# LuletterSoul/RP-Style-Transfer

Hardware: AMD Instinct MI355X
Metric: stylized images/sec at 512×512, 1/2/4/8 MI355X; % HBM roofline (higher is better)
Workload: dtype fp32

## Files before the change

rp-style-transfer_amd/csrc/rpst_wino4q.hip:

```cpp
#include "rpst_conv.h"

#include <type_traits>

#ifndef RPST_W4Q_DBG
#define RPST_W4Q_DBG 0
#endif

namespace rpst {
namespace {

template <int PAD>
__device__ __forceinline__ void q_mfma(floatx4& acc, float a, float b) {
  if constexpr (PAD)
    asm volatile("s_nop 1\n\tv_mfma_f32_16x16x4_f32 %0, %1, %2, %0" : "+v"(acc) : "v"(a), "v"(b));
  else
    asm volatile("v_mfma_f32_16x16x4_f32 %0, %1, %2, %0" : "+v"(acc) : "v"(a), "v"(b));
}
__device__ __forceinline__ unsigned q_lds_addr(const float* p) {
  return (unsigned)(uintptr_t)(const __attribute__((address_space(3))) float*)p;
}
template <int OFF>
__device__ __forceinline__ void q_dma16(__amdgpu_buffer_rsrc_t r, unsigned m0, unsigned voff,
                                        int soff) {
  asm volatile("s_mov_b32 m0, %0\n\ts_nop 0\n\tbuffer_load_dwordx4 %1, %2, %3 offen offset:%4 lds"
               :: "s"(m0), "v"(voff), "s"(r), "s"(soff), "i"(OFF) : "memory");
}
__device__ __forceinline__ void q_dma4(__amdgpu_buffer_rsrc_t r, unsigned m0, unsigned voff,
                                       int soff) {
  asm volatile("s_mov_b32 m0, %0\n\ts_nop 0\n\tbuffer_load_dword %1, %2, %3 offen lds"
               :: "s"(m0), "v"(voff), "s"(r), "s"(soff) : "memory");
}
__device__ __forceinline__ void q_lds_barrier() {
  asm volatile("s_waitcnt lgkmcnt(0)" ::: "memory");
  __builtin_amdgcn_s_barrier();
}

template <int H>
__device__ __forceinline__ void q_bt3(float d0, float d1, float d2, float d3, float d4, float d5,
                                      float& u0, float& u1, float& u2) {
  if constexpr (H == 0) {
    const float A = fmaf(-4.f, d2, d4), B = fmaf(-4.f, d1, d3);
    u0 = fmaf(4.f, d0, fmaf(-5.f, d2, d4));
    u1 = A + B;
    u2 = A - B;
  } else {
    const float C = d4 - d2, E = d3 - d1;
    u0 = fmaf(2.f, E, C);
    u1 = fmaf(-2.f, E, C);
    u2 = fmaf(4.f, d1, fmaf(-5.f, d3, d5));
  }
}

}

constexpr int kQCo = 64;
constexpr int kQTH = 8, kQTW = 64;
constexpr int kQXO = 4;
constexpr int kQPS = 72;
constexpr int kQCS = 768;
constexpr int kQWS = 9216;
constexpr int kQPAT = 4 * kQCS;
constexpr int kQNTH = 512;
constexpr int kQMaxCo = 512;
constexpr int kQWPI = 5;
constexpr int kQWide = 2, kQSlow = 6;
constexpr int kQDMA4 = 3, kQDMA = 12;
constexpr int kQRP = kQPS / 4;
constexpr int kQXS = 4 * 3 * 3 * 64 * 2;
constexpr int kQWG0 = 0;
constexpr int kQPG = 5;
constexpr int kQAhead = 3;
static_assert(10 * kQRP <= kQDMA4 * 64 && kQDMA4 * 256 <= kQCS, "16-B pieces in a channel");
static_assert(10 * kQPS <= kQDMA * 64 && kQDMA * 64 <= kQCS, "4-B pieces in a channel");
static_assert(2 * kQWide >= kQDMA4 && 2 * kQSlow >= kQDMA && 8 * kQWPI >= 36, "coverage");
static_assert(2 * kQXS <= kQWS, "the exchange fits a weight stage");
static_assert((2 * kQWS + 4 * kQPAT) * 4 + 1024 + kQSlow * kQNTH * 4 + 9 * kQMaxCo * 4 <= 163840,
              "LDS");

template <typename TW>
__global__ void wino4q_pack_kernel(const TW* __restrict__ w, float* __restrict__ pk, int Cout,
                                   int Cin, int K4, int64_t per, int64_t total, int64_t sco,
                                   int64_t sci, int64_t stap) {
  int64_t t = (int64_t)blockIdx.x * blockDim.x + threadIdx.x;
  if (t >= total) return;
  const int64_t img = t / per;
  pk += img * per;
  w += img * (int64_t)Cout * Cin * 9;
  t -= img * per;
  const int cb = (int)(t & 3);
  int64_t r = t >> 2;
  const int l = (int)(r & 63);
  r >>= 6;
  const int p = (int)(r % 9);
  r /= 9;
  const int q = (int)(r & 3);
  r >>= 2;
  const int ks = (int)(r % K4);
  const int ct = (int)(r / K4);
  const int i = 3 * (q >> 1) + p / 3, jj = 3 * (q & 1) + p % 3;
  const int co = ct * kQCo + cb * 16 + (l & 15);
  const int ci = ks * 4 + (l >> 4);
  float v = 0.f;
  if (co < Cout && ci < Cin) {
    const double G[6][3] = {{0.25, 0, 0},
                            {-1.0 / 6, -1.0 / 6, -1.0 / 6},
                            {-1.0 / 6, 1.0 / 6, -1.0 / 6},
                            {1.0 / 24, 1.0 / 12, 1.0 / 6},
                            {1.0 / 24, -1.0 / 12, 1.0 / 6},
                            {0, 0, 1}};
    const TW* g = w + co * sco + ci * sci;
    double acc = 0.0;
#pragma unroll
    for (int u = 0; u < 3; ++u)
#pragma unroll
      for (int s = 0; s < 3; ++s) acc += G[i][u] * (double)g[(u * 3 + s) * stap] * G[jj][s];
    v = (float)acc;
  }
  pk[t] = v;
}

size_t wino4q_packed_floats(int Cout, int Cin) {
  return (size_t)((Cout + kQCo - 1) / kQCo) * ((Cin + 3) / 4) * kQWS;
}

int wino4q_pack(const float* w, float* pk, int Cout, int Cin, hipStream_t st) {
  const int64_t t = (int64_t)wino4q_packed_floats(Cout, Cin);
  wino4q_pack_kernel<float><<<(unsigned)((t + 255) / 256), 256, 0, st>>>(
      w, pk, Cout, Cin, (Cin + 3) / 4, t, t, (int64_t)Cin * 9, 9, 1);
  return launch_status("wino4q_pack_kernel");
}

int wino4q_pack_mix(const double* wm, float* pk, int N, int Cout, int Cin, hipStream_t st) {
  const int64_t per = (int64_t)wino4q_packed_floats(Cout, Cin), tot = (int64_t)N * per;
  wino4q_pack_kernel<double><<<(unsigned)((tot + 255) / 256), 256, 0, st>>>(
      wm, pk, Cout, Cin, (Cin + 3) / 4, per, tot, Cin, 1, (int64_t)Cout * Cin);
  return launch_status("wino4q_pack_kernel(mix)");
}

__global__ void wino4q_fold_w_kernel(const float4* __restrict__ pk, float4* __restrict__ out,
                                     const float* __restrict__ aux, int N, int Cin, int K4,
                                     int64_t per4) {
  const int64_t t = (int64_t)blockIdx.x * blockDim.x + threadIdx.x;
  if (t >= (int64_t)N * per4) return;
  const int n = (int)(t / per4);
  const int64_t u = t - (int64_t)n * per4;
  const int l = (int)(u & 63);
  const int ks = (int)((u / (kQWS / 4)) % K4);
  const int ci = ks * 4 + (l >> 4);
  const int64_t nc = (int64_t)N * Cin, i = (int64_t)n * Cin + (ci < Cin ? ci : 0);
  const float sc = ci < Cin ? aux[3 * nc + i] / aux[2 * nc + i] : 0.f;
  const float4 v = pk[u];
  out[t] = make_float4(v.x * sc, v.y * sc, v.z * sc, v.w * sc);
}

int wino4q_fold_w(const float* pk, float* out, const float* aux, int N, int Cout, int Cin,
                  hipStream_t st) {
  const int64_t per4 = (int64_t)wino4q_packed_floats(Cout, Cin) / 4, n4 = (int64_t)N * per4;
  wino4q_fold_w_kernel<<<(unsigned)((n4 + 255) / 256), 256, 0, st>>>(
      reinterpret_cast<const float4*>(pk), reinterpret_cast<float4*>(out), aux, N, Cin,
      (Cin + 3) / 4, per4);
  return launch_status("wino4q_fold_w_kernel");
}

bool wino4q_applies(int Cin, int Cout, int in_op, const ConvMode& m) {
  const int min_cin = m.quarter == 2 ? 16 : 128;
  return m.quarter && m.precise != 2 && (in_op == RPST_IN_NONE || in_op == RPST_IN_UPSAMPLE2) &&
         Cout >= 64 && Cout <= kQMaxCo &&
         Cin >= min_cin && Cin % 16 == 0;
}

ConvTiling wino4q_tiling(ConvArgs& a) {
  a.Cout_pad = (a.Cout + kQCo - 1) / kQCo * kQCo;
  a.nchunks = (a.Cin + 3) / 4;
  a.tiles_x = (a.W + kQTW - 1) / kQTW;
  a.tiles_y = (a.H + kQTH - 1) / kQTH;
  a.co_tiles = a.Cout_pad / kQCo;
  a.stat_P = a.tiles_x * a.tiles_y * 2;
  a.cosplit = 1;
  return {(int64_t)a.tiles_x * a.tiles_y * a.N, kQNTH, 4, kQTH / 4, kQTW, true};
}

struct QEpi {
  int W, H, Cout, gy0, gx0, rows, n, sidx;
  bool vec, full, bst, edge, store, pool;
  float inv, slope;
  unsigned voff[4];
  float* out;
  float* oimg;
  unsigned obytes;
  const float* btab;
  float2* statp;
  int statP;
};

__device__ __forceinline__ QEpi q_epi_ctx(int wr, int tn) {
  const KArgs L = late_args();
  QEpi e;
  e.W = L->W;
  e.H = L->H;
  e.Cout = L->Cout;
  e.slope = L->relu == RPST_ACT_RELU ? 0.f : (L->relu == RPST_ACT_LRELU ? 0.2f : 1.f);
  int btx, bty;
  w4_tile((int)blockIdx.x / L->cosplit, L->tiles_x, L->tiles_y, btx, bty, e.n);
  const int bx0 = btx * kQTW;
  e.gy0 = bty * kQTH + 4 * wr;
  e.gx0 = bx0 + 4 * tn;
  e.vec = (e.W & 3) == 0 && e.gx0 + 3 < e.W;
  e.rows = max(0, min(4, e.H - e.gy0));
  const int cols = max(0, min(kQTW, e.W - bx0));
  e.inv = e.rows * cols > 0 ? __builtin_amdgcn_rcpf((float)(e.rows * cols)) : 0.f;
  e.full = e.rows == 4 && bx0 + kQTW <= e.W;
  e.edge = e.gy0 == 0 || e.gy0 + 4 >= e.H || bx0 == 0 || bx0 + kQTW >= e.W;
  e.out = L->out;
  const int64_t plane = (int64_t)e.H * e.W;
  e.pool = L->pool_out != 0;
  e.bst = !e.pool && (e.W & 3) == 0 && (int64_t)e.Cout * plane * 4 < (1LL << 31);
  e.oimg = e.out + (int64_t)e.n * e.Cout * plane;
  const bool keep = L->skip_from <= 0 || e.n < L->skip_from;
  e.obytes = keep ? (unsigned)(e.Cout * plane * 4) : 0u;
  e.store = keep;
#pragma unroll
  for (int yy = 0; yy < 4; ++yy)
    e.voff[yy] = (yy < e.rows && e.gx0 < e.W) ? (unsigned)(((e.gy0 + yy) * e.W + e.gx0) * 4)
                                             : 0x80000000u;
  e.btab = L->btab;
  e.statp = L->stat_part;
  e.statP = L->stat_P;
  e.sidx = (bty * L->tiles_x + btx) * 2 + wr;
  return e;
}

template <bool STATS, bool BTAB, bool RELU>
__device__ __forceinline__ void q_finish(const QEpi& e, int co, float (&Y)[16], int tn) {
  const int gy0 = e.gy0, gx0 = e.gx0, rows = e.rows, n = e.n;
  const bool cok = co < e.Cout;
  if constexpr (BTAB) {
    if (e.edge) {
      const float* bt = e.btab + (cok ? co : 0) * 9;
      float b9[9];
#pragma unroll
      for (int i = 0; i < 9; ++i) b9[i] = cok ? bt[i] : 0.f;
      const float b4 = b9[4];
#pragma unroll
      for (int i = 0; i < 9; ++i) b9[i] -= b4;
#pragma unroll
      for (int yy = 0; yy < 4; ++yy) {
        const int gy = gy0 + yy;
        const int rc = gy == 0 ? 0 : (gy >= e.H - 1 ? 2 : 1);
        const float l = rc == 0 ? b9[0] : (rc == 2 ? b9[6] : b9[3]);
        const float m = rc == 0 ? b9[1] : (rc == 2 ? b9[7] : b9[4]);
        const float r = rc == 0 ? b9[2] : (rc == 2 ? b9[8] : b9[5]);
#pragma unroll
        for (int xx = 0; xx < 4; ++xx) {
          const int gx = gx0 + xx;
          Y[yy * 4 + xx] += gx == 0 ? l : (gx >= e.W - 1 ? r : m);
        }
      }
    }
  }
#pragma unroll
  for (int i = 0; i < 16; ++i)
    Y[i] = __builtin_amdgcn_fmed3f(Y[i], RELU ? 0.f : e.slope * Y[i], __builtin_inff());
  float sum = 0.f;
  if constexpr (STATS) {
    if (e.full) {
#pragma unroll
      for (int i = 0; i < 16; ++i) sum += Y[i];
    } else {
#pragma unroll
      for (int yy = 0; yy < 4; ++yy)
#pragma unroll
        for (int xx = 0; xx < 4; ++xx) sum += (yy < rows && gx0 + xx < e.W) ? Y[yy * 4 + xx] : 0.f;
    }
  }
  if ((RPST_W4Q_DBG & 64) && e.statP > -7) {
  } else if (e.bst) {
    const auto ro = rsrc_or_zero(e.oimg, e.obytes, true);
    const unsigned cofs = cok ? (unsigned)co * (unsigned)(e.H * e.W) * 4u : 0x7fffffffu;
#pragma unroll
    for (int yy = 0; yy < 4; ++yy) {
      const floatx4 v = {Y[yy * 4], Y[yy * 4 + 1], Y[yy * 4 + 2], Y[yy * 4 + 3]};
      __builtin_amdgcn_raw_buffer_store_b128(__builtin_bit_cast(u32x4, v), ro,
                                             (int)(e.voff[yy] + cofs), 0, 0);
    }
  } else if (e.pool) {
    if (cok && e.store) {
      const int Ho = (e.H + 1) >> 1, Wo = (e.W + 1) >> 1;
      float* o = e.out + (((int64_t)n * e.Cout + co) * Ho + (gy0 >> 1)) * Wo + (gx0 >> 1);
#pragma unroll
      for (int py = 0; py < 2; ++py) {
        if (2 * py >= rows) continue;
        const bool y1 = 2 * py + 1 < rows;
        float pv[2];
#pragma unroll
        for (int px = 0; px < 2; ++px) {
          const bool x1 = gx0 + 2 * px + 1 < e.W;
          const float* t = Y + (2 * py) * 4 + 2 * px;
          float v = t[0];
          if (x1) v = fmaxf(v, t[1]);
          if (y1) v = fmaxf(v, t[4]);
          if (x1 && y1) v = fmaxf(v, t[5]);
          pv[px] = v;
        }
        if (gx0 + 3 < e.W && (Wo & 1) == 0) {
          *reinterpret_cast<float2*>(o + py * Wo) = make_float2(pv[0], pv[1]);
        } else {
          if (gx0 < e.W) o[py * Wo] = pv[0];
          if (gx0 + 2 < e.W) o[py * Wo + 1] = pv[1];
        }
      }
    }
  } else if (cok && e.store) {
    float* o = e.out + (((int64_t)n * e.Cout + co) * e.H + gy0) * e.W + gx0;
#pragma unroll
    for (int yy = 0; yy < 4; ++yy) {
      if (yy < rows) {
        if (e.vec) {
          *reinterpret_cast<float4*>(o + yy * e.W) =
              make_float4(Y[yy * 4], Y[yy * 4 + 1], Y[yy * 4 + 2], Y[yy * 4 + 3]);
        } else {
#pragma unroll
          for (int xx = 0; xx < 4; ++xx)
            if (gx0 + xx < e.W) o[yy * e.W + xx] = Y[yy * 4 + xx];
        }
      }
    }
  }
  if constexpr (STATS) {
    sum = row16_sum(sum);
    const float mean = sum * e.inv;
    float m2 = 0.f;
    if (e.full) {
#pragma unroll
      for (int i = 0; i < 16; ++i) m2 = fmaf(Y[i] - mean, Y[i] - mean, m2);
    } else {
#pragma unroll
      for (int yy = 0; yy < 4; ++yy)
#pragma unroll
        for (int xx = 0; xx < 4; ++xx) {
          const float dv = Y[yy * 4 + xx] - mean;
          m2 += (yy < rows && gx0 + xx < e.W) ? dv * dv : 0.f;
        }
    }
    m2 = row16_sum(m2);
    if (tn == 0 && cok)
      e.statp[((int64_t)n * e.statP + e.sidx) * e.Cout + co] = make_float2(mean, m2);
  }
}

template <int INOP, bool STATS, bool BTAB, bool RELU>
__global__ __launch_bounds__(kQNTH, 1) void wino4q_mfma_kernel(ConvArgs a) {
  __shared__ __attribute__((aligned(16))) float ws0[kQWS];
  __shared__ __attribute__((aligned(16))) float ws1[kQWS];
  __shared__ __attribute__((aligned(16))) float ps0[kQPAT];
  __shared__ __attribute__((aligned(16))) float ps1[kQPAT];
  __shared__ __attribute__((aligned(16))) float ps2[kQPAT];
  __shared__ __attribute__((aligned(16))) float ps3[kQPAT];
  __shared__ __attribute__((aligned(16))) float dummy[256];
  __shared__ unsigned poffs[kQSlow][kQNTH];
  __shared__ float btl[BTAB ? 9 * kQMaxCo : kQMaxCo];

  const int wave = __builtin_amdgcn_readfirstlane((int)threadIdx.x >> 6);
  const int lane = threadIdx.x & 63;
  const int k = lane >> 4, tn = lane & 15, wr = wave >> 2;

  int bid = (int)blockIdx.x;
  const int cog = bid % a.cosplit;
  bid /= a.cosplit;
  const int nct = a.co_tiles / a.cosplit, ct0 = cog * nct;
  int tx, ty, n;
  w4_tile(bid, a.tiles_x, a.tiles_y, tx, ty, n);
  const int K4 = a.nchunks, G = nct * K4;
  const int y0 = ty * kQTH, x0 = tx * kQTW;

  {
    const int nb = BTAB ? 9 * a.Cout : a.Cout;
    const float* src = BTAB ? a.btab + (int64_t)n * nb : a.bias;
    for (int i = threadIdx.x; i < nb; i += kQNTH) btl[i] = src ? src[i] : 0.f;
  }
  constexpr bool up = INOP == RPST_IN_UPSAMPLE2;
  const unsigned in_plane = up ? (unsigned)(a.Hs * a.Ws) : (unsigned)(a.H * a.W);
  const unsigned oob = a.Cin * in_plane * 4u;
  const float* in_img = conv_in_img(a, n, (int64_t)a.Cin * in_plane);
  const unsigned wbytes = (unsigned)(nct * K4 * kQWS) * 4u;
  const float* w_img = a.wpk + (int64_t)n * a.wstride + (int64_t)ct0 * K4 * kQWS;

  const int hf = wave & 1;
  const bool zp = a.pad == RPST_PAD_ZERO;
  const int rs = up ? a.Ws : a.W;
  const bool w4a = (a.W & 3) == 0;
  const bool wide = !up && ((x0 >= 1 && x0 + kQTW < a.W) || (w4a && x0 + kQTW <= a.W));
  const bool fixL = wide && w4a && !zp && x0 == 0;
  const bool fixR = wide && w4a && !zp && x0 + kQTW == a.W;
  unsigned poff[kQSlow];
  const int tid = threadIdx.x;
  if (wide) {
#pragma unroll
    for (int i = 0; i < kQWide; ++i) {
      const int p = kQWide * hf + i;
      const int f = 64 * p + lane, row = min(f / kQRP, 9), j = f - (f / kQRP) * kQRP;
      int y = y0 - 1 + row;
      const int xs = x0 - kQXO + 4 * j;
      const bool okx = !w4a || (xs >= 0 && xs + 3 < a.W);
      const bool ok = p < kQDMA4 && f < 10 * kQRP && resolve_bf(y, a.H, zp) && okx;
      poff[i] = ok ? ((unsigned)(y * rs) + (unsigned)xs) * 4u : oob;
    }
#pragma unroll
    for (int i = kQWide; i < kQSlow; ++i) poff[i] = oob;
  } else {
#pragma unroll
    for (int i = 0; i < kQSlow; ++i) {
      const int p = kQSlow * hf + i;
      const int f = 64 * p + lane;
      const int row = min(f / kQPS, 9), col = f - (f / kQPS) * kQPS;
      int y = y0 - 1 + row, x = x0 - kQXO + col;
      const bool oky = resolve_bf(y, a.H, zp), okx = resolve_bf(x, a.W, zp);
      const bool ok = p < kQDMA && col >= kQXO - 1 && col < kQXO + 1 + kQTW &&
                      f < 10 * kQPS && oky && okx;
      poff[i] = ok ? ((unsigned)((up ? y >> 1 : y) * rs) + (unsigned)(up ? x >> 1 : x)) * 4u : oob;
    }
  }
#pragma unroll
  for (int i = 0; i < kQSlow; ++i) poffs[i][tid] = poff[i];

  constexpr int DBG = RPST_W4Q_DBG;
  const int wl = wave * 4096;
  const bool real4 = wave < 4;
  const int w4 = 32768 + wave * 1024;
  const unsigned dummy_a = q_lds_addr(dummy);
  int wso = wl;
  auto issue_w = [&](bool live, unsigned stg, auto Ic) {
    constexpr int I = decltype(Ic)::value;
    if (DBG & 2) return;
    if constexpr (I < 4) {
      q_dma16<1024 * I>(rsrc_or_zero(w_img, wbytes, live), stg + wl, lane * 16, wso);
    } else {
      q_dma16<0>(rsrc_or_zero(w_img, wbytes, live && real4), real4 ? stg + w4 : dummy_a,
                 lane * 16, wso + (w4 - wl));
    }
  };
  const unsigned pstep = 4u * in_plane * 4u;
  const int pbase = (int)((unsigned)(wave >> 1) * in_plane * 4u);
  const bool h1 = (wave & 1) != 0;
  const int pl = (wave >> 1) * (kQCS * 4) + (h1 ? (wide ? 2048 : kQSlow * 256) : 0);
  int pso = pbase;
  auto issue_p = [&](auto WIDEc, bool live, unsigned stg) {
    constexpr bool WIDE = decltype(WIDEc)::value;
    if (DBG & 1) return;
    const auto r = rsrc_or_zero(in_img, oob, live);
    const unsigned xs = stg + launder(pl);
    if constexpr (WIDE) {
      q_dma16<0>(r, xs, poffs[0][tid], pso);
      q_dma16<0>(r, h1 ? dummy_a : xs + 1024, poffs[1][tid], pso);
    } else {
#pragma unroll
      for (int i = 0; i < kQSlow; ++i) q_dma4(r, xs + 256 * i, poffs[i][tid], pso);
    }
    pso += (int)pstep;
  };
  const bool bst_all = !a.pool_out && (a.W & 3) == 0 &&
                       (int64_t)a.Cout * a.H * a.W * 4 < (1LL << 31);
  bool post_epi = false;
  auto wait_ring = [&](bool first) {
    if (DBG & 128) return;
    if (first && post_epi && bst_all) {
      if (wide) asm volatile("s_waitcnt vmcnt(18)" ::: "memory");
      else asm volatile("s_waitcnt vmcnt(22)" ::: "memory");
    } else if (wide) {
      asm volatile("s_waitcnt vmcnt(2)" ::: "memory");
    } else {
      asm volatile("s_waitcnt vmcnt(6)" ::: "memory");
    }
    if (first) post_epi = false;
  };

  auto fix_halo = [&](float* stg) {
    if ((wave == 0 && fixL) || (wave == 1 && fixR)) {
      int l = lane;
      asm volatile("" : "+v"(l));
      if (l < 40) {
        const int ch = l / 10, row = l - 10 * ch;
        float* rp = stg + ch * kQCS + row * kQPS;
        if (wave == 0) rp[kQXO - 1] = rp[kQXO + 1];
        else rp[kQXO + kQTW] = rp[kQXO + kQTW - 2];
      }
    }
  };
  auto prologue = [&](auto WIDEc) {
    issue_p(WIDEc, true, q_lds_addr(ps0));
    issue_p(WIDEc, true, q_lds_addr(ps1));
    issue_w(true, q_lds_addr(ws0), std::integral_constant<int, 0>{});
    issue_w(true, q_lds_addr(ws0), std::integral_constant<int, 1>{});
    issue_w(true, q_lds_addr(ws0), std::integral_constant<int, 2>{});
    issue_w(true, q_lds_addr(ws0), std::integral_constant<int, 3>{});
    issue_w(true, q_lds_addr(ws0), std::integral_constant<int, 4>{});
    issue_p(WIDEc, true, q_lds_addr(ps2));
    issue_p(WIDEc, true, q_lds_addr(ps3));
  };
  if (wide) prologue(std::true_type{});
  else prologue(std::false_type{});
  wait_ring(false);
  q_lds_barrier();
  if (fixL || fixR) {
    fix_halo(ps0);
    fix_halo(ps1);
    q_lds_barrier();
  }

  auto body = [&](auto Qc) {
    constexpr int Q = decltype(Qc)::value, QR = Q >> 1, QC = Q & 1;
    floatx4 acc[9][4];
#pragma unroll
    for (int p = 0; p < 9; ++p)
#pragma unroll
      for (int cb = 0; cb < 4; ++cb) acc[p][cb] = floatx4{0.f, 0.f, 0.f, 0.f};
    const int roff = k * kQCS + (4 * wr + QR) * kQPS + 4 * tn;
    auto read_row = [&](const float* stg, int rr, float (&d)[8]) {
      const float* rp = stg + roff + rr * kQPS;
      floatx4 u = *reinterpret_cast<const floatx4*>(rp + 4);
      const float e = QC ? rp[8] : rp[3];
      asm("" : "+v"(u));
      d[0] = QC ? 0.f : e; d[1] = u[0]; d[2] = u[1]; d[3] = u[2]; d[4] = u[3];
      d[5] = QC ? e : 0.f; d[6] = 0.f; d[7] = 0.f;
    };
    auto col_pass = [&](const float (&d)[8], float (&u)[3]) {
      if (DBG & 8) {
        u[0] = d[0]; u[1] = d[1]; u[2] = d[2];
        return;
      }
      q_bt3<QC>(d[0], d[1], d[2], d[3], d[4], d[5], u[0], u[1], u[2]);
    };
    auto row_pass = [&](const float (&u)[5][3], int j, float (&v)[9]) {
      if (DBG & 8) {
        v[j] = u[0][j]; v[3 + j] = u[2][j]; v[6 + j] = u[4][j];
        return;
      }
      if constexpr (QR == 0)
        q_bt3<0>(u[0][j], u[1][j], u[2][j], u[3][j], u[4][j], 0.f, v[j], v[3 + j], v[6 + j]);
      else
        q_bt3<1>(0.f, u[0][j], u[1][j], u[2][j], u[3][j], u[4][j], v[j], v[3 + j], v[6 + j]);
    };
    float V[9];
    {
      float u[5][3];
#pragma unroll
      for (int rr = 0; rr < 5; ++rr) {
        float d[8];
        read_row(ps0, rr, d);
        col_pass(d, u[rr]);
      }
#pragma unroll
      for (int j = 0; j < 3; ++j) row_pass(u, j, V);
    }

    const int woff = Q * 9 * 256 + lane * 4;
    int x = 0;
    auto step = [&](float* wsx, float* psn, float* wsn, float* psx, float* pfx, int ks,
                    bool first) {
      wait_ring(first);
      const bool wlive = x + 1 < G, plive = x + 4 < G;
      wso += kQWS * 4;
      if (first && ks + 4 == K4) pso = pbase;
      const unsigned wsn_a = q_lds_addr(wsn), psx_a = q_lds_addr(psx);
      if (DBG & 16) asm volatile("s_waitcnt lgkmcnt(0)" ::: "memory");
      else q_lds_barrier();
      constexpr int ord[9] = {0, 3, 6, 1, 4, 7, 2, 5, 8};
      constexpr int kA = kQAhead;
      float4 w4[9];
#pragma unroll
      for (int q = 0; q < kA; ++q)
        w4[ord[q]] = *reinterpret_cast<const float4*>(wsx + woff + ord[q] * 256);
      float d[8];
      read_row(psn, 0, d);
      float u[5][3];
#pragma unroll
      for (int q = 0; q < 9; ++q) {
        const int p = ord[q];
        if (q + kA < 9)
          w4[ord[q + kA]] = *reinterpret_cast<const float4*>(wsx + woff + ord[q + kA] * 256);
        q_mfma<1>(acc[p][0], w4[p].x, V[p]);
        q_mfma<0>(acc[p][1], w4[p].y, V[p]);
        q_mfma<0>(acc[p][2], w4[p].z, V[p]);
        q_mfma<0>(acc[p][3], w4[p].w, V[p]);
        if (q == kQWG0) issue_w(wlive, wsn_a, std::integral_constant<int, 0>{});
        if (q == kQWG0 + 1) issue_w(wlive, wsn_a, std::integral_constant<int, 1>{});
        if (q == kQWG0 + 2) issue_w(wlive, wsn_a, std::integral_constant<int, 2>{});
        if (q == kQWG0 + 3) issue_w(wlive, wsn_a, std::integral_constant<int, 3>{});
        if (q == kQWG0 + 4) issue_w(wlive, wsn_a, std::integral_constant<int, 4>{});
        if (q == kQPG) {
          if (wide) issue_p(std::true_type{}, plive, psx_a);
          else issue_p(std::false_type{}, plive, psx_a);
        }
        if (q < 5) {
          col_pass(d, u[q]);
          if (q + 1 < 5) read_row(psn, q + 1, d);
        }
        if (q == 5 || q == 6 || q == 8) row_pass(u, q == 8 ? 2 : q - 5, V);
        if (q == 7) fix_halo(pfx);
      }
      ++x;
    };

    auto epilogue = [&](int ctile) {
      if (DBG & 32) {
        float t = 0.f;
#pragma unroll
        for (int p = 0; p < 9; ++p)
#pragma unroll
          for (int cb = 0; cb < 4; ++cb) t += acc[p][cb][0];
        if (t == 1.2345f) late_args()->out[threadIdx.x] = t;
#pragma unroll
        for (int p = 0; p < 9; ++p)
#pragma unroll
          for (int cb = 0; cb < 4; ++cb) acc[p][cb] = floatx4{0.f, 0.f, 0.f, 0.f};
        return;
      }
      q_lds_barrier();
      asm volatile("s_nop 7\n\ts_nop 4" : "+v"(acc[0][0]), "+v"(acc[0][1]), "+v"(acc[0][2]),
                   "+v"(acc[0][3]), "+v"(acc[1][0]), "+v"(acc[1][1]), "+v"(acc[1][2]),
                   "+v"(acc[1][3]), "+v"(acc[2][0]), "+v"(acc[2][1]), "+v"(acc[2][2]),
                   "+v"(acc[2][3]), "+v"(acc[3][0]), "+v"(acc[3][1]), "+v"(acc[3][2]),
                   "+v"(acc[3][3]), "+v"(acc[4][0]), "+v"(acc[4][1]));
      asm volatile("" : "+v"(acc[4][2]), "+v"(acc[4][3]), "+v"(acc[5][0]), "+v"(acc[5][1]),
                   "+v"(acc[5][2]), "+v"(acc[5][3]), "+v"(acc[6][0]), "+v"(acc[6][1]),
                   "+v"(acc[6][2]), "+v"(acc[6][3]), "+v"(acc[7][0]), "+v"(acc[7][1]),
                   "+v"(acc[7][2]), "+v"(acc[7][3]), "+v"(acc[8][0]), "+v"(acc[8][1]),
                   "+v"(acc[8][2]), "+v"(acc[8][3]));
      const int co0 = ctile * kQCo + 16 * Q + 4 * k;
#pragma unroll
      for (int rp = 0; rp < 2; ++rp) {
        float P[2][6][4];
#pragma unroll
        for (int pt = 0; pt < 3; ++pt) {
          float* xb = ws1 + wr * kQXS;
#pragma unroll
          for (int dq = 0; dq < 4; ++dq) {
            if (dq == Q || (DBG & 4)) continue;
            const int slot = (Q - dq - 1) & 3;
#pragma unroll
            for (int j = 0; j < 3; ++j)
              *reinterpret_cast<float2*>(xb + (((dq * 3 + slot) * 3 + j) * 64 + lane) * 2) =
                  make_float2(acc[3 * pt + j][dq][2 * rp], acc[3 * pt + j][dq][2 * rp + 1]);
          }
          if (!(DBG & 4)) q_lds_barrier();
          float m[2][2][6];
#pragma unroll
          for (int s = 0; s < 4; ++s) {
#pragma unroll
            for (int j = 0; j < 3; ++j) {
              float2 v;
              if (s == Q || (DBG & 4)) {
                const int src = (DBG & 4) ? s : Q;
                v = make_float2(acc[3 * pt + j][src][2 * rp], acc[3 * pt + j][src][2 * rp + 1]);
              } else {
                v = *reinterpret_cast<const float2*>(
                    xb + (((Q * 3 + ((s - Q - 1) & 3)) * 3 + j) * 64 + lane) * 2);
              }
              m[0][s >> 1][3 * (s & 1) + j] = v.x;
              m[1][s >> 1][3 * (s & 1) + j] = v.y;
            }
          }
#pragma unroll
          for (int e2 = 0; e2 < 2; ++e2) {
            at6(m[e2][0], P[e2][pt]);
            at6(m[e2][1], P[e2][3 + pt]);
          }
          if (!(DBG & 4) && (rp == 0 || pt < 2)) q_lds_barrier();
        }
#pragma unroll
        for (int e2 = 0; e2 < 2; ++e2) {
          const int r = 2 * rp + e2;
          QEpi e = q_epi_ctx(wr, tn);
          e.btab = btl;
          float bias = 0.f;
          {
            const int co = co0 + r;
            if (co < e.Cout) bias = BTAB ? btl[co * 9 + 4] : btl[co];
          }
#pragma unroll
          for (int x = 0; x < 4; ++x) P[e2][1][x] += bias;
          float Y[16];
#pragma unroll
          for (int x = 0; x < 4; ++x) {
            float c6[6], y[4];
#pragma unroll
            for (int I = 0; I < 6; ++I) c6[I] = P[e2][I][x];
            at6(c6, y);
#pragma unroll
            for (int yy = 0; yy < 4; ++yy) Y[yy * 4 + x] = y[yy];
          }
          q_finish<STATS, BTAB, RELU>(e, co0 + r, Y, tn);
        }
      }
#pragma unroll
      for (int p = 0; p < 9; ++p)
#pragma unroll
        for (int cb = 0; cb < 4; ++cb) acc[p][cb] = floatx4{0.f, 0.f, 0.f, 0.f};
    };

    int ks = 0, ct = ct0;
    for (int g = 0; g < G; g += 4) {
      step(ws0, ps1, ws1, ps0, ps2, ks, true);
      step(ws1, ps2, ws0, ps1, ps3, ks + 1, false);
      step(ws0, ps3, ws1, ps2, ps0, ks + 2, false);
      step(ws1, ps0, ws0, ps3, ps1, ks + 3, false);
      ks += 4;
      if (ks == K4) {
        epilogue(ct);
        post_epi = true;
        ks = 0;
        ++ct;
      }
    }
  };
  switch (wave & 3) {
    case 0: body(std::integral_constant<int, 0>{}); break;
    case 1: body(std::integral_constant<int, 1>{}); break;
    case 2: body(std::integral_constant<int, 2>{}); break;
    default: body(std::integral_constant<int, 3>{}); break;
  }
  asm volatile("s_waitcnt vmcnt(0)" ::: "memory");
}

int wino4q_launch(ConvArgs& a, int in_op, hipStream_t st) {
  RPST_REQUIRE(in_op == RPST_IN_NONE || in_op == RPST_IN_UPSAMPLE2,
               "conv2d: winograd4 (quarter) does not support in_op %d", in_op);
  const ConvTiling t = wino4q_tiling(a);
  RPST_REQUIRE((int64_t)a.co_tiles * a.nchunks * kQWS * 4 < (1LL << 31),
               "conv2d: winograd4 weight image exceeds 2 GiB");
  RPST_REQUIRE(t.blocks <= 0x7fffffffLL, "conv2d: grid too large");
  const unsigned nb = (unsigned)t.blocks;
  const bool stats = a.stat_part != nullptr, btab = a.btab != nullptr;
  RPST_REQUIRE(!btab || in_op == RPST_IN_NONE, "conv2d: winograd4 bias table with a loader op");
  RPST_REQUIRE(!(stats && btab), "conv2d: winograd4 folded bias with statistics");
#define RPST_W4Q_GO(OP, S, B)                                                  \
  do {                                                                         \
    if (a.relu == RPST_ACT_RELU)                                               \
      wino4q_mfma_kernel<OP, S, B, true><<<nb, kQNTH, 0, st>>>(a);             \
    else                                                                       \
      wino4q_mfma_kernel<OP, S, B, false><<<nb, kQNTH, 0, st>>>(a);            \
  } while (0)
  if (in_op == RPST_IN_UPSAMPLE2) {
    if (stats) RPST_W4Q_GO(RPST_IN_UPSAMPLE2, true, false);
    else RPST_W4Q_GO(RPST_IN_UPSAMPLE2, false, false);
  } else {
    if (stats) RPST_W4Q_GO(RPST_IN_NONE, true, false);
    else if (btab) RPST_W4Q_GO(RPST_IN_NONE, false, true);
    else RPST_W4Q_GO(RPST_IN_NONE, false, false);
  }
#undef RPST_W4Q_GO
  return launch_status("wino4q_mfma_kernel");
}

}
```

Measured before the change: 570.6.

## Precompute epilogue context into LDS and rematerialize lane ids to cut register pressure

Replaces the per-call epilogue context (recomputed from kernel args for each output channel and held in registers) with a per-block record and per-lane store offsets. The first 32 threads fill these into shared memory once, and q_finish reads them from LDS with readfirstlane-uniformized pointers. Lane, tid and k/tn are recomputed via mbcnt right where they are needed, so these values do not stay live across the MFMA main loop. The goal is fewer live VGPRs and less scalar/vector work per epilogue. In exchange the epilogue does extra LDS reads and the kernel uses 1 KB more shared memory.

```diff
diff --git a/rp-style-transfer_amd/csrc/rpst_wino4q.hip b/rp-style-transfer_amd/csrc/rpst_wino4q.hip
--- a/rp-style-transfer_amd/csrc/rpst_wino4q.hip
+++ b/rp-style-transfer_amd/csrc/rpst_wino4q.hip
@@ -29,6 +29,13 @@
                                        int soff) {
   asm volatile("s_mov_b32 m0, %0\n\ts_nop 0\n\tbuffer_load_dword %1, %2, %3 offen lds"
                :: "s"(m0), "v"(voff), "s"(r), "s"(soff) : "memory");
+}
+__device__ __forceinline__ int q_lane_here() {
+  int z = 0;
+#if __HIP_DEVICE_COMPILE__
+  asm volatile("" : "+v"(z));
+#endif
+  return (int)__builtin_amdgcn_mbcnt_hi(~0u, __builtin_amdgcn_mbcnt_lo(~0u, (unsigned)z));
 }
 __device__ __forceinline__ void q_lds_barrier() {
   asm volatile("s_waitcnt lgkmcnt(0)" ::: "memory");
@@ -74,7 +81,9 @@
 static_assert(10 * kQPS <= kQDMA * 64 && kQDMA * 64 <= kQCS, "4-B pieces in a channel");
 static_assert(2 * kQWide >= kQDMA4 && 2 * kQSlow >= kQDMA && 8 * kQWPI >= 36, "coverage");
 static_assert(2 * kQXS <= kQWS, "the exchange fits a weight stage");
-static_assert((2 * kQWS + 4 * kQPAT) * 4 + 1024 + kQSlow * kQNTH * 4 + 9 * kQMaxCo * 4 <= 163840,
+constexpr int kQEpiB = 1024;
+static_assert((2 * kQWS + 4 * kQPAT) * 4 + 1024 + kQSlow * kQNTH * 4 + 9 * kQMaxCo * 4 + kQEpiB <=
+                  163840,
               "LDS");
 
 template <typename TW>
@@ -180,63 +189,80 @@
   return {(int64_t)a.tiles_x * a.tiles_y * a.N, kQNTH, 4, kQTH / 4, kQTW, true};
 }
 
-struct QEpi {
-  int W, H, Cout, gy0, gx0, rows, n, sidx;
-  bool vec, full, bst, edge, store, pool;
+struct QEpiRec {
+  float* oimg;
+  float* out;
+  float2* stat;
+  unsigned obytes;
+  unsigned hw4;
+  int W, H, Cout, gy0, bx0, rows, n;
+  unsigned flags;
   float inv, slope;
-  unsigned voff[4];
-  float* out;
-  float* oimg;
-  unsigned obytes;
-  const float* btab;
-  float2* statp;
-  int statP;
 };
-
-__device__ __forceinline__ QEpi q_epi_ctx(int wr, int tn) {
-  const KArgs L = late_args();
-  QEpi e;
-  e.W = L->W;
-  e.H = L->H;
-  e.Cout = L->Cout;
-  e.slope = L->relu == RPST_ACT_RELU ? 0.f : (L->relu == RPST_ACT_LRELU ? 0.2f : 1.f);
-  int btx, bty;
-  w4_tile((int)blockIdx.x / L->cosplit, L->tiles_x, L->tiles_y, btx, bty, e.n);
-  const int bx0 = btx * kQTW;
-  e.gy0 = bty * kQTH + 4 * wr;
-  e.gx0 = bx0 + 4 * tn;
-  e.vec = (e.W & 3) == 0 && e.gx0 + 3 < e.W;
-  e.rows = max(0, min(4, e.H - e.gy0));
-  const int cols = max(0, min(kQTW, e.W - bx0));
-  e.inv = e.rows * cols > 0 ? __builtin_amdgcn_rcpf((float)(e.rows * cols)) : 0.f;
-  e.full = e.rows == 4 && bx0 + kQTW <= e.W;
-  e.edge = e.gy0 == 0 || e.gy0 + 4 >= e.H || bx0 == 0 || bx0 + kQTW >= e.W;
-  e.out = L->out;
-  const int64_t plane = (int64_t)e.H * e.W;
-  e.pool = L->pool_out != 0;
-  e.bst = !e.pool && (e.W & 3) == 0 && (int64_t)e.Cout * plane * 4 < (1LL << 31);
-  e.oimg = e.out + (int64_t)e.n * e.Cout * plane;
-  const bool keep = L->skip_from <= 0 || e.n < L->skip_from;
-  e.obytes = keep ? (unsigned)(e.Cout * plane * 4) : 0u;
-  e.store = keep;
+constexpr unsigned kQFFull = 1, kQFEdge = 2, kQFBst = 4, kQFPool = 8, kQFStore = 16;
+typedef float floatx2 __attribute__((ext_vector_type(2)));
+typedef __attribute__((address_space(1))) float gfloat;
+typedef __attribute__((address_space(1))) floatx2 gfloatx2;
+typedef __attribute__((address_space(1))) floatx4 gfloatx4;
+static_assert(2 * (sizeof(QEpiRec) + 15) / 16 * 16 + 2 * 16 * 16 <= kQEpiB, "LDS");
+
+__device__ __forceinline__ void q_epi_fill(const ConvArgs& a, int tx, int ty, int n, int t,
+                                           QEpiRec* recs, uint4* voffs) {
+  const int wr = t >> 4, tn = t & 15;
+  const int bx0 = tx * kQTW, gy0 = ty * kQTH + 4 * wr, gx0 = bx0 + 4 * tn;
+  const int rows = max(0, min(4, a.H - gy0));
+  unsigned vo[4];
 #pragma unroll
   for (int yy = 0; yy < 4; ++yy)
-    e.voff[yy] = (yy < e.rows && e.gx0 < e.W) ? (unsigned)(((e.gy0 + yy) * e.W + e.gx0) * 4)
-                                             : 0x80000000u;
-  e.btab = L->btab;
-  e.statp = L->stat_part;
-  e.statP = L->stat_P;
-  e.sidx = (bty * L->tiles_x + btx) * 2 + wr;
-  return e;
+    vo[yy] = (yy < rows && gx0 < a.W) ? (unsigned)(((gy0 + yy) * a.W + gx0) * 4) : 0x80000000u;
+  voffs[t] = make_uint4(vo[0], vo[1], vo[2], vo[3]);
+  if (tn) return;
+  QEpiRec r;
+  r.W = a.W;
+  r.H = a.H;
+  r.Cout = a.Cout;
+  r.gy0 = gy0;
+  r.bx0 = bx0;
+  r.rows = rows;
+  r.n = n;
+  r.slope = a.relu == RPST_ACT_RELU ? 0.f : (a.relu == RPST_ACT_LRELU ? 0.2f : 1.f);
+  const int cols = max(0, min(kQTW, a.W - bx0));
+  r.inv = rows * cols > 0 ? __builtin_amdgcn_rcpf((float)(rows * cols)) : 0.f;
+  const int64_t plane = (int64_t)a.H * a.W;
+  const bool full = rows == 4 && bx0 + kQTW <= a.W;
+  const bool edge = gy0 == 0 || gy0 + 4 >= a.H || bx0 == 0 || bx0 + kQTW >= a.W;
+  const bool pool = a.pool_out != 0;
+  const bool bst = !pool && (a.W & 3) == 0 && (int64_t)a.Cout * plane * 4 < (1LL << 31);
+  const bool keep = a.skip_from <= 0 || n < a.skip_from;
+  r.flags = (full ? kQFFull : 0u) | (edge ? kQFEdge : 0u) | (bst ? kQFBst : 0u) |
+            (pool ? kQFPool : 0u) | (keep ? kQFStore : 0u);
+  r.out = a.out;
+  r.oimg = a.out + (int64_t)n * a.Cout * plane;
+  r.obytes = keep ? (unsigned)(a.Cout * plane * 4) : 0u;
+  r.hw4 = (unsigned)(a.H * a.W) * 4u;
+  const int sidx = (ty * a.tiles_x + tx) * 2 + wr;
+  r.stat = a.stat_part ? a.stat_part + ((int64_t)n * a.stat_P + sidx) * a.Cout : nullptr;
+  recs[wr] = r;
+}
+
+__device__ __forceinline__ unsigned uni(unsigned v) {
+  return (unsigned)__builtin_amdgcn_readfirstlane((int)v);
+}
+__device__ __forceinline__ float* uni(float* p) {
+  const uint64_t u = (uint64_t)(uintptr_t)p;
+  return (float*)(uintptr_t)(((uint64_t)uni((unsigned)(u >> 32)) << 32) | uni((unsigned)u));
 }
 
 template <bool STATS, bool BTAB, bool RELU>
-__device__ __forceinline__ void q_finish(const QEpi& e, int co, float (&Y)[16], int tn) {
-  const int gy0 = e.gy0, gx0 = e.gx0, rows = e.rows, n = e.n;
-  const bool cok = co < e.Cout;
+__device__ __forceinline__ void q_finish(const QEpiRec& r, const uint4& vo, const float* btab,
+                                         int co, unsigned cofs, float (&Y)[16], int tn) {
+  const unsigned f = r.flags;
+  const bool full = (f & kQFFull) != 0;
+  const bool cok = co < r.Cout;
   if constexpr (BTAB) {
-    if (e.edge) {
-      const float* bt = e.btab + (cok ? co : 0) * 9;
+    if (f & kQFEdge) {
+      const int gy0 = r.gy0, gx0 = r.bx0 + 4 * tn, H = r.H, W = r.W;
+      const float* bt = btab + (cok ? co : 0) * 9;
       float b9[9];
 #pragma unroll
       for (int i = 0; i < 9; ++i) b9[i] = cok ? bt[i] : 0.f;
@@ -246,47 +272,57 @@
 #pragma unroll
       for (int yy = 0; yy < 4; ++yy) {
         const int gy = gy0 + yy;
-        const int rc = gy == 0 ? 0 : (gy >= e.H - 1 ? 2 : 1);
+        const int rc = gy == 0 ? 0 : (gy >= H - 1 ? 2 : 1);
         const float l = rc == 0 ? b9[0] : (rc == 2 ? b9[6] : b9[3]);
         const float m = rc == 0 ? b9[1] : (rc == 2 ? b9[7] : b9[4]);
-        const float r = rc == 0 ? b9[2] : (rc == 2 ? b9[8] : b9[5]);
+        const float rr = rc == 0 ? b9[2] : (rc == 2 ? b9[8] : b9[5]);
 #pragma unroll
         for (int xx = 0; xx < 4; ++xx) {
           const int gx = gx0 + xx;
-          Y[yy * 4 + xx] += gx == 0 ? l : (gx >= e.W - 1 ? r : m);
+          Y[yy * 4 + xx] += gx == 0 ? l : (gx >= W - 1 ? rr : m);
         }
       }
     }
   }
-#pragma unroll
-  for (int i = 0; i < 16; ++i)
-    Y[i] = __builtin_amdgcn_fmed3f(Y[i], RELU ? 0.f : e.slope * Y[i], __builtin_inff());
+  if constexpr (RELU) {
+#pragma unroll
+    for (int i = 0; i < 16; ++i) Y[i] = __builtin_amdgcn_fmed3f(Y[i], 0.f, __builtin_inff());
+  } else {
+    const float slope = r.slope;
+#pragma unroll
+    for (int i = 0; i < 16; ++i)
+      Y[i] = __builtin_amdgcn_fmed3f(Y[i], slope * Y[i], __builtin_inff());
+  }
   float sum = 0.f;
   if constexpr (STATS) {
-    if (e.full) {
+    if (full) {
 #pragma unroll
       for (int i = 0; i < 16; ++i) sum += Y[i];
     } else {
+      const int rows = r.rows, gx0 = r.bx0 + 4 * tn, W = r.W;
 #pragma unroll
       for (int yy = 0; yy < 4; ++yy)
 #pragma unroll
-        for (int xx = 0; xx < 4; ++xx) sum += (yy < rows && gx0 + xx < e.W) ? Y[yy * 4 + xx] : 0.f;
-    }
-  }
-  if ((RPST_W4Q_DBG & 64) && e.statP > -7) {
-  } else if (e.bst) {
-    const auto ro = rsrc_or_zero(e.oimg, e.obytes, true);
-    const unsigned cofs = cok ? (unsigned)co * (unsigned)(e.H * e.W) * 4u : 0x7fffffffu;
+        for (int xx = 0; xx < 4; ++xx) sum += (yy < rows && gx0 + xx < W) ? Y[yy * 4 + xx] : 0.f;
+    }
+  }
+  if ((RPST_W4Q_DBG & 64) && r.H > -7) {
+  } else if (f & kQFBst) {
+    const auto ro = rsrc_or_zero(uni(r.oimg), uni(r.obytes), true);
+    const unsigned chofs = cok ? cofs : 0x7fffffffu;
+    const unsigned voff[4] = {vo.x, vo.y, vo.z, vo.w};
 #pragma unroll
     for (int yy = 0; yy < 4; ++yy) {
       const floatx4 v = {Y[yy * 4], Y[yy * 4 + 1], Y[yy * 4 + 2], Y[yy * 4 + 3]};
       __builtin_amdgcn_raw_buffer_store_b128(__builtin_bit_cast(u32x4, v), ro,
-                                             (int)(e.voff[yy] + cofs), 0, 0);
-    }
-  } else if (e.pool) {
-    if (cok && e.store) {
-      const int Ho = (e.H + 1) >> 1, Wo = (e.W + 1) >> 1;
-      float* o = e.out + (((int64_t)n * e.Cout + co) * Ho + (gy0 >> 1)) * Wo + (gx0 >> 1);
+                                             (int)(voff[yy] + chofs), 0, 0);
+    }
+  } else if (f & kQFPool) {
+    if (cok && (f & kQFStore)) {
+      const int gy0 = r.gy0, gx0 = r.bx0 + 4 * tn, rows = r.rows, H = r.H, W = r.W;
+      const int Ho = (H + 1) >> 1, Wo = (W + 1) >> 1;
+      gfloat* o = (gfloat*)r.out + (((int64_t)r.n * r.Cout + co) * Ho + (gy0 >> 1)) * Wo +
+                  (gx0 >> 1);
 #pragma unroll
       for (int py = 0; py < 2; ++py) {
         if (2 * py >= rows) continue;
@@ -294,7 +330,7 @@
         float pv[2];
 #pragma unroll
         for (int px = 0; px < 2; ++px) {
-          const bool x1 = gx0 + 2 * px + 1 < e.W;
+          const bool x1 = gx0 + 2 * px + 1 < W;
           const float* t = Y + (2 * py) * 4 + 2 * px;
           float v = t[0];
           if (x1) v = fmaxf(v, t[1]);
@@ -302,49 +338,51 @@
           if (x1 && y1) v = fmaxf(v, t[5]);
           pv[px] = v;
         }
-        if (gx0 + 3 < e.W && (Wo & 1) == 0) {
-          *reinterpret_cast<float2*>(o + py * Wo) = make_float2(pv[0], pv[1]);
+        if (gx0 + 3 < W && (Wo & 1) == 0) {
+          *(gfloatx2*)(o + py * Wo) = floatx2{pv[0], pv[1]};
         } else {
-          if (gx0 < e.W) o[py * Wo] = pv[0];
-          if (gx0 + 2 < e.W) o[py * Wo + 1] = pv[1];
+          if (gx0 < W) o[py * Wo] = pv[0];
+          if (gx0 + 2 < W) o[py * Wo + 1] = pv[1];
         }
       }
     }
-  } else if (cok && e.store) {
-    float* o = e.out + (((int64_t)n * e.Cout + co) * e.H + gy0) * e.W + gx0;
+  } else if (cok && (f & kQFStore)) {
+    const int gy0 = r.gy0, gx0 = r.bx0 + 4 * tn, rows = r.rows, H = r.H, W = r.W;
+    const bool vec = (W & 3) == 0 && gx0 + 3 < W;
+    gfloat* o = (gfloat*)r.out + (((int64_t)r.n * r.Cout + co) * H + gy0) * W + gx0;
 #pragma unroll
     for (int yy = 0; yy < 4; ++yy) {
       if (yy < rows) {
-        if (e.vec) {
-          *reinterpret_cast<float4*>(o + yy * e.W) =
-              make_float4(Y[yy * 4], Y[yy * 4 + 1], Y[yy * 4 + 2], Y[yy * 4 + 3]);
+        if (vec) {
+          *(gfloatx4*)(o + yy * W) =
+              floatx4{Y[yy * 4], Y[yy * 4 + 1], Y[yy * 4 + 2], Y[yy * 4 + 3]};
         } else {
 #pragma unroll
           for (int xx = 0; xx < 4; ++xx)
-            if (gx0 + xx < e.W) o[yy * e.W + xx] = Y[yy * 4 + xx];
+            if (gx0 + xx < W) o[yy * W + xx] = Y[yy * 4 + xx];
         }
       }
     }
   }
   if constexpr (STATS) {
     sum = row16_sum(sum);
-    const float mean = sum * e.inv;
+    const float mean = sum * r.inv;
     float m2 = 0.f;
-    if (e.full) {
+    if (full) {
 #pragma unroll
       for (int i = 0; i < 16; ++i) m2 = fmaf(Y[i] - mean, Y[i] - mean, m2);
     } else {
+      const int rows = r.rows, gx0 = r.bx0 + 4 * tn, W = r.W;
 #pragma unroll
       for (int yy = 0; yy < 4; ++yy)
 #pragma unroll
         for (int xx = 0; xx < 4; ++xx) {
           const float dv = Y[yy * 4 + xx] - mean;
-          m2 += (yy < rows && gx0 + xx < e.W) ? dv * dv : 0.f;
+          m2 += (yy < rows && gx0 + xx < W) ? dv * dv : 0.f;
         }
     }
     m2 = row16_sum(m2);
-    if (tn == 0 && cok)
-      e.statp[((int64_t)n * e.statP + e.sidx) * e.Cout + co] = make_float2(mean, m2);
+    if (tn == 0 && cok) ((gfloatx2*)r.stat)[co] = floatx2{mean, m2};
   }
 }
 
@@ -361,8 +399,8 @@
   __shared__ float btl[BTAB ? 9 * kQMaxCo : kQMaxCo];
 
   const int wave = __builtin_amdgcn_readfirstlane((int)threadIdx.x >> 6);
-  const int lane = threadIdx.x & 63;
-  const int k = lane >> 4, tn = lane & 15, wr = wave >> 2;
+  int lane = threadIdx.x & 63;
+  const int wr = wave >> 2;
 
   int bid = (int)blockIdx.x;
   const int cog = bid % a.cosplit;
@@ -378,6 +416,9 @@
     const float* src = BTAB ? a.btab + (int64_t)n * nb : a.bias;
     for (int i = threadIdx.x; i < nb; i += kQNTH) btl[i] = src ? src[i] : 0.f;
   }
+  __shared__ __attribute__((aligned(16))) QEpiRec erec[2];
+  __shared__ uint4 evoff[2 * 16];
+  if (threadIdx.x < 32) q_epi_fill(a, tx, ty, n, (int)threadIdx.x, erec, evoff);
   constexpr bool up = INOP == RPST_IN_UPSAMPLE2;
   const unsigned in_plane = up ? (unsigned)(a.Hs * a.Ws) : (unsigned)(a.H * a.W);
   const unsigned oob = a.Cin * in_plane * 4u;
@@ -393,7 +434,7 @@
   const bool fixL = wide && w4a && !zp && x0 == 0;
   const bool fixR = wide && w4a && !zp && x0 + kQTW == a.W;
   unsigned poff[kQSlow];
-  const int tid = threadIdx.x;
+  int tid = threadIdx.x;
   if (wide) {
 #pragma unroll
     for (int i = 0; i < kQWide; ++i) {
@@ -476,8 +517,7 @@
 
   auto fix_halo = [&](float* stg) {
     if ((wave == 0 && fixL) || (wave == 1 && fixR)) {
-      int l = lane;
-      asm volatile("" : "+v"(l));
+      const int l = q_lane_here();
       if (l < 40) {
         const int ch = l / 10, row = l - 10 * ch;
         float* rp = stg + ch * kQCS + row * kQPS;
@@ -509,6 +549,9 @@
 
   auto body = [&](auto Qc) {
     constexpr int Q = decltype(Qc)::value, QR = Q >> 1, QC = Q & 1;
+    lane = q_lane_here();
+    tid = wave * 64 + lane;
+    const int k = lane >> 4, tn = lane & 15;
     floatx4 acc[9][4];
 #pragma unroll
     for (int p = 0; p < 9; ++p)
@@ -626,7 +669,10 @@
                    "+v"(acc[6][2]), "+v"(acc[6][3]), "+v"(acc[7][0]), "+v"(acc[7][1]),
                    "+v"(acc[7][2]), "+v"(acc[7][3]), "+v"(acc[8][0]), "+v"(acc[8][1]),
                    "+v"(acc[8][2]), "+v"(acc[8][3]));
-      const int co0 = ctile * kQCo + 16 * Q + 4 * k;
+      const int el = q_lane_here(), ek = el >> 4, etn = el & 15;
+      const int co0 = ctile * kQCo + 16 * Q + 4 * ek;
+      unsigned cofs = (unsigned)co0 * erec[wr].hw4;
+      asm volatile("" : "+v"(cofs));
 #pragma unroll
       for (int rp = 0; rp < 2; ++rp) {
         float P[2][6][4];
@@ -639,7 +685,7 @@
             const int slot = (Q - dq - 1) & 3;
 #pragma unroll
             for (int j = 0; j < 3; ++j)
-              *reinterpret_cast<float2*>(xb + (((dq * 3 + slot) * 3 + j) * 64 + lane) * 2) =
+              *reinterpret_cast<float2*>(xb + (((dq * 3 + slot) * 3 + j) * 64 + el) * 2) =
                   make_float2(acc[3 * pt + j][dq][2 * rp], acc[3 * pt + j][dq][2 * rp + 1]);
           }
           if (!(DBG & 4)) q_lds_barrier();
@@ -654,7 +700,7 @@
                 v = make_float2(acc[3 * pt + j][src][2 * rp], acc[3 * pt + j][src][2 * rp + 1]);
               } else {
                 v = *reinterpret_cast<const float2*>(
-                    xb + (((Q * 3 + ((s - Q - 1) & 3)) * 3 + j) * 64 + lane) * 2);
+                    xb + (((Q * 3 + ((s - Q - 1) & 3)) * 3 + j) * 64 + el) * 2);
               }
               m[0][s >> 1][3 * (s & 1) + j] = v.x;
               m[1][s >> 1][3 * (s & 1) + j] = v.y;
@@ -670,12 +716,10 @@
 #pragma unroll
         for (int e2 = 0; e2 < 2; ++e2) {
           const int r = 2 * rp + e2;
-          QEpi e = q_epi_ctx(wr, tn);
-          e.btab = btl;
           float bias = 0.f;
           {
             const int co = co0 + r;
-            if (co < e.Cout) bias = BTAB ? btl[co * 9 + 4] : btl[co];
+            if (co < erec[wr].Cout) bias = BTAB ? btl[co * 9 + 4] : btl[co];
           }
 #pragma unroll
           for (int x = 0; x < 4; ++x) P[e2][1][x] += bias;
@@ -689,7 +733,8 @@
 #pragma unroll
             for (int yy = 0; yy < 4; ++yy) Y[yy * 4 + x] = y[yy];
           }
-          q_finish<STATS, BTAB, RELU>(e, co0 + r, Y, tn);
+          q_finish<STATS, BTAB, RELU>(erec[wr], evoff[wr * 16 + etn], btl, co0 + r, cofs, Y, etn);
+          cofs += erec[wr].hw4;
         }
       }
 #pragma unroll
```

Result: faster. 582.7, median of 6 (+2.1%).
